# arkworks-rs/crypto-primitives

Measured on NVIDIA B200. Metric: poseidon_perms_per_sec, higher is better.
Workload: dtype u32x8 (256-bit Montgomery integer)

## Files before the change

### crypto_primitives_b200/csrc/cpb_poseidon.cu

```cuda
#include <cstdlib>
#include <vector>

#include "poseidon_kernels.cuh"

namespace cpb {

std::string& last_error_ref() {
    static thread_local std::string s;
    return s;
}
cpb_status fail(cpb_status st, const char* fmt, ...) {
    char buf[512];
    va_list ap;
    va_start(ap, fmt);
    vsnprintf(buf, sizeof buf, fmt, ap);
    va_end(ap);
    last_error_ref() = buf;
    return st;
}
void keep_pool_memory(int device) {
    cudaMemPool_t pool = nullptr;
    if (cudaDeviceGetDefaultMemPool(&pool, device) == cudaSuccess && pool) {
        unsigned long long keep = ~0ull;
        cudaMemPoolSetAttribute(pool, cudaMemPoolAttrReleaseThreshold, &keep);
    }
    cudaGetLastError();
}
int sm_count(int device) {
    static int cache[64];
    static std::mutex mu;
    std::lock_guard<std::mutex> g(mu);
    if (device < 0 || device >= 64) return 148;
    if (!cache[device]) {
        int v = 0;
        if (cudaDeviceGetAttribute(&v, cudaDevAttrMultiProcessorCount, device) != cudaSuccess || v <= 0) v = 148;
        cache[device] = v;
    }
    return cache[device];
}

template <class F>
__global__ void k_field_convert(const u32* __restrict__ in, u32* __restrict__ out, long n, int to_mont) {
    long i = (long)blockIdx.x * blockDim.x + threadIdx.x;
    if (i >= n) return;
    u32 a[8], k[8];
    ld_elem(a, in + 8 * i);
    if (to_mont) {
        for (int it = 0; it < 18; it++) {
            u32 t[8];
            t[0] = sub_cc(a[0], F::P(0));
#pragma unroll
            for (int j = 1; j < 8; j++) t[j] = subc_cc(a[j], F::P(j));
            u32 borrow = subc(0, 0);
            if (borrow) break;
            fp_copy(a, t);
        }
#pragma unroll
        for (int j = 0; j < 8; j++) k[j] = F::R2(j);
    } else {
        fp_zero(k);
        k[0] = 1;
    }
    u32 pm[8];
    fp_modulus<F>(pm);
    fp_mul<F>(a, a, k, pm);
    st_elem(out + 8 * i, a);
}

}

using namespace cpb;

using namespace cpb;

namespace cpb {
CPB_POS_WIDTHS(CPB_POS_EXTERN, Bls12_381_Fr)
CPB_POS_WIDTHS(CPB_POS_EXTERN, Bn254_Fr)
CPB_POS_WIDTHS(CPB_POS_EXTERN, Jubjub_Fr)
CPB_POS_WIDTHS(CPB_POS_EXTERN, Bls12_377_Fr)
CPB_POS_EXTERN_TEAM(Bls12_381_Fr)
CPB_POS_EXTERN_TEAM(Bn254_Fr)
CPB_POS_EXTERN_TEAM(Jubjub_Fr)
CPB_POS_EXTERN_TEAM(Bls12_377_Fr)
}

namespace {

PoseidonDev to_dev(const host::PoseidonSchedule& S) {
    PoseidonDev D;
    D.t = S.t; D.rate = S.rate; D.cap = S.capacity; D.rf = S.rf; D.rp = S.rp; D.sparse = S.sparse; D.alpha = S.alpha;
    D.off_c = S.off_c; D.off_m = S.off_m; D.off_mpre = S.off_mpre; D.off_cp0 = S.off_cp0; D.off_pc = S.off_pc;
    D.off_sp = S.off_sp; D.off_arkp = S.off_arkp; D.off_mod = S.off_mod; D.off_sc0 = S.off_sc0; D.n_elems = S.n_elems; D.zero = 0;
    return D;
}


#define CPB_CASE_T(F, T, M, ...) case T: return M<F, T>(__VA_ARGS__);
#define CPB_FOR_T(F, M, ...)                                                                                   \
    switch (c->dev.t) {                                                                                        \
        CPB_CASE_T(F, 2, M, __VA_ARGS__) CPB_CASE_T(F, 3, M, __VA_ARGS__) CPB_CASE_T(F, 4, M, __VA_ARGS__)     \
        CPB_CASE_T(F, 5, M, __VA_ARGS__) CPB_CASE_T(F, 6, M, __VA_ARGS__) CPB_CASE_T(F, 7, M, __VA_ARGS__)     \
        CPB_CASE_T(F, 8, M, __VA_ARGS__) CPB_CASE_T(F, 9, M, __VA_ARGS__)                                      \
    }                                                                                                          \
    break;
#define CPB_FOR_FIELD(M, ...)                                                        \
    switch (c->field_id) {                                                           \
        case CPB_BLS12_381_FR: CPB_FOR_T(Bls12_381_Fr, M, __VA_ARGS__)               \
        case CPB_BN254_FR: CPB_FOR_T(Bn254_Fr, M, __VA_ARGS__)                       \
        case CPB_JUBJUB_FR: CPB_FOR_T(Jubjub_Fr, M, __VA_ARGS__)                     \
        case CPB_BLS12_377_FR: CPB_FOR_T(Bls12_377_Fr, M, __VA_ARGS__)               \
    }

size_t team_max() {
    static long v = -1;
    if (v < 0) {
        const char* e = getenv("CPB_TEAM_MAX");
        v = e ? atol(e) : 4096;
        if (v > 4096) v = 4096;
        if (v < 0) v = 0;
    }
    return (size_t)v;
}
size_t team_max_for(size_t S) {
    if (getenv("CPB_TEAM_MAX")) return team_max();
    size_t v = 8192 / (S ? S : 1);
    return v < team_max() ? v : team_max();
}
bool team_capable(const cpb_poseidon_ctx* c) { return c->dev.t == 3 && c->dev.cap == 1 && c->dev.alpha >= 2; }

cpb_status launch_tree_top(cpb_poseidon_ctx* c, const TopJob& J, cudaStream_t st) {
    switch (c->field_id) {
        case CPB_BLS12_381_FR: return launch_tree_top_f<Bls12_381_Fr>(c, J, st);
        case CPB_BN254_FR: return launch_tree_top_f<Bn254_Fr>(c, J, st);
        case CPB_JUBJUB_FR: return launch_tree_top_f<Jubjub_Fr>(c, J, st);
        case CPB_BLS12_377_FR: return launch_tree_top_f<Bls12_377_Fr>(c, J, st);
    }
    return fail(CPB_BAD_PARAMS, "unknown field id %d", c->field_id);
}

}

namespace cpb {
cpb_status launch_crh(cpb_poseidon_ctx* c, const u32* in, size_t len, u32* out, size_t n, cudaStream_t st, size_t n_out) {
    if (n == 0 || n_out == 0) return CPB_OK;
    if (team_capable(c) && len == 2 && n_out == 1 && n <= team_max()) {
        TopJob J;
        J.flat_in = in; J.flat_out = out; J.n_flat = (long)n;
        return launch_tree_top(c, J, st);
    }
    CPB_FOR_FIELD(launch_crh_ft, c, in, len, out, n_out, n, st)
    return fail(CPB_UNSUPPORTED, "state width t=%d is not built (this library: t = 2..9)", c->dev.t);
}
}

namespace {
cpb_status launch_verify(cpb_poseidon_ctx* c, cpb_poseidon_ctx* node, const u32* root, const u32* leaves, size_t leaf_len,
                         const u32* siblings, const u32* paths, int plen, const unsigned long long* indexes, unsigned char* ok,
                         size_t n, cudaStream_t st) {
    if (n == 0) return CPB_OK;
    CPB_FOR_FIELD(launch_verify_ft, c, node, root, leaves, leaf_len, siblings, paths, plen, indexes, ok, n, st)
    return fail(CPB_UNSUPPORTED, "state width t=%d is not built (this library: t = 2..9)", c->dev.t);
}
cpb_status launch_permute(cpb_poseidon_ctx* c, const u32* in, u32* out, size_t n, cudaStream_t st) {
    if (n == 0) return CPB_OK;
    CPB_FOR_FIELD(launch_permute_ft, c, in, out, n, st)
    return fail(CPB_UNSUPPORTED, "state width t=%d is not built (this library: t = 2..9)", c->dev.t);
}

}

namespace cpb {

cpb_status check_ctx(const cpb_poseidon_ctx* c) {
    if (!c) return fail(CPB_NULL_POINTER, "null context");
    return CPB_OK;
}

cpb_status merkle_subtree_levels(cpb_poseidon_ctx* node, const u32* leaf_digests, size_t n, u32* nodes, size_t S, size_t k,
                                 cudaStream_t st, const MerkleHost* H, const ExchangeDev* X, int* small_from) {
    int h = 0;
    while (((size_t)1 << h) < n) h++;
    int lg = 0;
    while (((size_t)1 << lg) < S) lg++;
    const bool team = team_capable(node) && team_max() > 0;
    const size_t tmax = team_max_for(S);
    for (int l = h - 1; l >= lg; l--) {
        size_t cnt = ((size_t)1 << l) / S;
        if (team && cnt <= tmax) {
            TopJob J;
            J.leaf_digests = leaf_digests; J.nodes = nodes; J.h = h; J.lgS = lg; J.k = (long)k; J.l_start = l; J.l_end = lg;
            if (X && S == 1) J.x = *X;
            CPB_TRY(launch_tree_top(node, J, st));
            if (small_from) *small_from = l;
            else if (H)
                for (int q = l; q >= lg; q--) {
                    size_t c2 = ((size_t)1 << q) / S, off = (((size_t)1 << q) - 1) + k * c2;
                    CPB_CUDA(cudaMemcpyAsync(H->node_ptr(q, k * c2), nodes + 8 * off, c2 * 32, cudaMemcpyDeviceToHost, st));
                }
            return CPB_OK;
        }
        const u32* in = (l == h - 1) ? leaf_digests + 8 * (2 * k * cnt) : nodes + 8 * ((((size_t)1 << (l + 1)) - 1) + 2 * k * cnt);
        u32* out = nodes + 8 * ((((size_t)1 << l) - 1) + k * cnt);
        CPB_TRY(launch_crh(node, in, 2, out, cnt, st));
        if (H) CPB_CUDA(cudaMemcpyAsync(H->node_ptr(l, k * cnt), out, cnt * 32, cudaMemcpyDeviceToHost, st));
    }
    if (X && S == 1) return fail(CPB_UNSUPPORTED, "the fused root exchange needs a rate-2, capacity-1 Poseidon two-to-one hash with alpha >= 2");
    return CPB_OK;
}
cpb_status merkle_levels(cpb_poseidon_ctx* node, const u32* leaf_digests, size_t n, u32* nodes, cudaStream_t st) {
    return merkle_subtree_levels(node, leaf_digests, n, nodes, 1, 0, st);
}

size_t merkle_streams(size_t n) {
    static int forced = -1;
    if (forced < 0) {
        const char* e = getenv("CPB_MERKLE_STREAMS");
        forced = e ? atoi(e) : 0;
    }
    size_t S = forced > 0 ? (size_t)forced : 8;
    if (S > 8) S = 8;
    while (S & (S - 1)) S &= S - 1;
    while (S > 1 && n / S < ((size_t)1 << 14)) S >>= 1;
    return S;
}

cpb_status ensure_side_streams(cpb_poseidon_ctx* c, size_t S) {
    std::lock_guard<std::mutex> lk(c->side_mu);
    for (size_t i = 0; i < S; i++)
        if (!c->side[i]) CPB_CUDA(cudaStreamCreateWithFlags(&c->side[i], cudaStreamNonBlocking));
    return CPB_OK;
}

cpb_status merkle_build_streams(cpb_poseidon_ctx* leaf, cpb_poseidon_ctx* node, const u32* leaves, size_t leaf_len, size_t n,
                                u32* leaf_nodes, u32* nodes, cudaStream_t st, const MerkleHost* H, const ExchangeDev* X) {
    size_t S = merkle_streams(n);
    if (S <= 1) {
        if (H && H->leaves && n * leaf_len) CPB_CUDA(cudaMemcpyAsync((void*)leaves, H->leaves, n * leaf_len * 32, cudaMemcpyHostToDevice, st));
        if (leaves) CPB_TRY(launch_crh(leaf, leaves, leaf_len, leaf_nodes, n, st));
        CPB_TRY(merkle_subtree_levels(node, leaf_nodes, n, nodes, 1, 0, st, H, X));
        if (H) CPB_CUDA(cudaMemcpyAsync(H->leaf_nodes, leaf_nodes, n * 32, cudaMemcpyDeviceToHost, st));
        return CPB_OK;
    }
    CPB_TRY(ensure_side_streams(node, S));
    int small_from = -1;
    cudaEvent_t start = nullptr, done[8] = {};
    CPB_CUDA(cudaEventCreateWithFlags(&start, cudaEventDisableTiming));
    cudaError_t e = cudaEventRecord(start, st);
    cpb_status rc = CPB_OK;
// ... 103 lines not shown
    if (!ptr) return fail(CPB_NULL_POINTER, "null buffer");
    CPB_CUDA(cudaHostUnregister(ptr));
    return CPB_OK;
    });
}

cpb_status cpb_field_modulus(int field_id, uint64_t out[4]) {
    return cpb::guarded([&]() -> cpb_status {
    const uint64_t* m = host::field_modulus(field_id);
    if (!m) return fail(CPB_BAD_PARAMS, "unknown field id %d", field_id);
    if (!out) return fail(CPB_NULL_POINTER, "null out");
    memcpy(out, m, 32);
    return CPB_OK;
    });
}

static cpb_status field_convert(int field_id, int device, const uint64_t* in, uint64_t* out, size_t n, int to_mont) {
    if (!host::field_modulus(field_id)) return fail(CPB_BAD_PARAMS, "unknown field id %d", field_id);
    if (n == 0) return CPB_OK;
    if (!in || !out) return fail(CPB_NULL_POINTER, "null buffer");
    DeviceGuard g(device);
    if (!g.ok) return fail(CPB_NO_DEVICE, "cudaSetDevice(%d) failed", device);
    u32* d = nullptr;
    CPB_CUDA(cudaMalloc(&d, n * 32));
    cudaError_t e = cudaMemcpy(d, in, n * 32, cudaMemcpyHostToDevice);
    if (e == cudaSuccess) {
        int grid = (int)((n + 127) / 128);
        switch (field_id) {
            case 0: k_field_convert<Bls12_381_Fr><<<grid, 128>>>(d, d, (long)n, to_mont); break;
            case 1: k_field_convert<Bn254_Fr><<<grid, 128>>>(d, d, (long)n, to_mont); break;
            case 2: k_field_convert<Jubjub_Fr><<<grid, 128>>>(d, d, (long)n, to_mont); break;
            case 3: k_field_convert<Bls12_377_Fr><<<grid, 128>>>(d, d, (long)n, to_mont); break;
        }
        e = cudaGetLastError();
    }
    if (e == cudaSuccess) e = cudaMemcpy(out, d, n * 32, cudaMemcpyDeviceToHost);
    cudaFree(d);
    if (e != cudaSuccess) return fail(CPB_CUDA_ERROR, "field conversion failed: %s", cudaGetErrorString(e));
    return CPB_OK;
}
static cpb_status field_convert_dev(int field_id, int device, const uint64_t* in, uint64_t* out, size_t n, int to_mont, void* stream) {
    if (!host::field_modulus(field_id)) return fail(CPB_BAD_PARAMS, "unknown field id %d", field_id);
    if (n == 0) return CPB_OK;
    if (!in || !out) return fail(CPB_NULL_POINTER, "null buffer");
    DeviceGuard g(device);
    if (!g.ok) return fail(CPB_NO_DEVICE, "cudaSetDevice(%d) failed", device);
    cudaStream_t st = (cudaStream_t)stream;
    const u32* d_in = (const u32*)in;
    u32* d_out = (u32*)out;
    long left = (long)n, off = 0;
    while (left > 0) {
        long m = left < (1L << 28) ? left : (1L << 28);
        int grid = (int)((m + 127) / 128);
        switch (field_id) {
            case 0: k_field_convert<Bls12_381_Fr><<<grid, 128, 0, st>>>(d_in + 8 * off, d_out + 8 * off, m, to_mont); break;
            case 1: k_field_convert<Bn254_Fr><<<grid, 128, 0, st>>>(d_in + 8 * off, d_out + 8 * off, m, to_mont); break;
            case 2: k_field_convert<Jubjub_Fr><<<grid, 128, 0, st>>>(d_in + 8 * off, d_out + 8 * off, m, to_mont); break;
            case 3: k_field_convert<Bls12_377_Fr><<<grid, 128, 0, st>>>(d_in + 8 * off, d_out + 8 * off, m, to_mont); break;
        }
        CPB_CUDA(cudaGetLastError());
        left -= m; off += m;
    }
    return CPB_OK;
}
cpb_status cpb_field_to_montgomery_dev(int field_id, int device, const uint64_t* in, uint64_t* out, size_t n, void* stream) {
    return cpb::guarded([&]() -> cpb_status { return field_convert_dev(field_id, device, in, out, n, 1, stream); });
}
cpb_status cpb_field_from_montgomery_dev(int field_id, int device, const uint64_t* in, uint64_t* out, size_t n, void* stream) {
    return cpb::guarded([&]() -> cpb_status { return field_convert_dev(field_id, device, in, out, n, 0, stream); });
}
cpb_status cpb_field_to_montgomery(int field_id, int device, const uint64_t* in, uint64_t* out, size_t n) {
    return cpb::guarded([&]() -> cpb_status {
    return field_convert(field_id, device, in, out, n, 1);
    });
}
cpb_status cpb_field_from_montgomery(int field_id, int device, const uint64_t* in, uint64_t* out, size_t n) {
    return cpb::guarded([&]() -> cpb_status {
    return field_convert(field_id, device, in, out, n, 0);
    });
}

cpb_status cpb_poseidon_find_ark_and_mds(int field_id, uint64_t prime_bits, int rate, int full_rounds,
                                         int partial_rounds, int skip_matrices, uint64_t* ark_out, uint64_t* mds_out) {
    return cpb::guarded([&]() -> cpb_status {
    const uint64_t* mod = host::field_modulus(field_id);
    if (!mod) return fail(CPB_BAD_PARAMS, "unknown field id %d", field_id);
    if (!ark_out || !mds_out) return fail(CPB_NULL_POINTER, "null output");
    host::Field F(mod);
    if (prime_bits != (uint64_t)F.bits)
        return fail(CPB_BAD_PARAMS, "prime_bits %llu != MODULUS_BIT_SIZE %d", (unsigned long long)prime_bits, F.bits);
    if (rate < 1 || rate > 15 || full_rounds < 0 || partial_rounds < 0 || full_rounds > 1023 || partial_rounds > 1023 ||
        skip_matrices < 0)
        return fail(CPB_BAD_PARAMS, "bad shape");
    host::FeVec ark, mds;
    host::find_poseidon_ark_and_mds(F, prime_bits, rate, full_rounds, partial_rounds, skip_matrices, ark, mds);
    memcpy(ark_out, ark.data(), ark.size() * 32);
    memcpy(mds_out, mds.data(), mds.size() * 32);
    return CPB_OK;
    });
}

cpb_status cpb_poseidon_default_entry(int field_id, int rate, int optimized_for_weights, uint64_t* alpha, int* full_rounds,
                                      int* partial_rounds, int* skip_matrices) {
    return cpb::guarded([&]() -> cpb_status {
    host::DefaultEntry e;
    if (!host::default_entry(field_id, rate, optimized_for_weights != 0, e))
        return fail(CPB_BAD_PARAMS, "no default entry for field %d rate %d", field_id, rate);
    if (alpha) *alpha = e.alpha;
    if (full_rounds) *full_rounds = e.rf;
    if (partial_rounds) *partial_rounds = e.rp;
    if (skip_matrices) *skip_matrices = e.skip;
    return CPB_OK;
    });
}

cpb_status cpb_poseidon_ctx_create(int field_id, int rate, int capacity, int full_rounds, int partial_rounds,
                                   uint64_t alpha, const uint64_t* ark, const uint64_t* mds, int device,
                                   cpb_poseidon_ctx** out) {
    return cpb::guarded([&]() -> cpb_status {
    if (!out) return fail(CPB_NULL_POINTER, "null out");
    *out = nullptr;
    const uint64_t* mod = host::field_modulus(field_id);
    if (!mod) return fail(CPB_BAD_PARAMS, "unknown field id %d", field_id);
    if (!ark || !mds) return fail(CPB_NULL_POINTER, "null ark/mds");
    if (rate < 1 || capacity < 1 || rate + capacity > 16 || full_rounds < 0 || partial_rounds < 0 ||
        full_rounds + partial_rounds < 1)
        return fail(CPB_BAD_PARAMS, "bad Poseidon shape rate=%d capacity=%d RF=%d RP=%d", rate, capacity, full_rounds,
                    partial_rounds);
    host::Field F(mod);
    host::PoseidonParams P;
    P.rate = rate; P.capacity = capacity; P.full_rounds = full_rounds; P.partial_rounds = partial_rounds; P.alpha = alpha;
    int t = rate + capacity;
    P.ark.resize((size_t)(full_rounds + partial_rounds) * t);
    P.mds.resize((size_t)t * t);
    memcpy(P.ark.data(), ark, P.ark.size() * 32);
    memcpy(P.mds.data(), mds, P.mds.size() * 32);
    for (const auto& e : P.ark)
        if (!F.is_canonical(e)) return fail(CPB_BAD_PARAMS, "ark element not reduced");
    for (const auto& e : P.mds)
        if (!F.is_canonical(e)) return fail(CPB_BAD_PARAMS, "mds element not reduced");

    DeviceGuard g(device);
    if (!g.ok) { cudaGetLastError(); return fail(CPB_NO_DEVICE, "cudaSetDevice(%d) failed: no usable CUDA device", device); }
    int major = 0;
    CPB_CUDA(cudaDeviceGetAttribute(&major, cudaDevAttrComputeCapabilityMajor, device));
    if (major != 10) return fail(CPB_NO_DEVICE, "device %d is sm_%d0; this library is built for sm_100a only", device, major);

    keep_pool_memory(device);
    cpb_poseidon_ctx* c = new cpb_poseidon_ctx();
    c->field_id = field_id;
    c->device = device;
    c->sms = sm_count(device);
    c->sched = host::derive_schedule(F, P, true);
    c->dev = to_dev(c->sched);
    size_t bytes = c->sched.consts.size() * 8;
    if (bytes > 200 * 1024) { delete c; return fail(CPB_UNSUPPORTED, "round schedule (%zu B) exceeds shared memory", bytes); }
    cudaError_t e = cudaMalloc(&c->d_consts, bytes);
    if (e == cudaSuccess) e = cudaMemcpy(c->d_consts, c->sched.consts.data(), bytes, cudaMemcpyHostToDevice);
    if (e == cudaSuccess) e = cudaStreamCreateWithFlags(&c->stream, cudaStreamNonBlocking);
    if (e != cudaSuccess) {
        if (c->d_consts) cudaFree(c->d_consts);
        delete c;
        return fail(CPB_CUDA_ERROR, "context upload failed: %s", cudaGetErrorString(e));
    }
    *out = c;
    return CPB_OK;
    });
}

void cpb_poseidon_ctx_destroy(cpb_poseidon_ctx* c) {
    if (!c) return;
    DeviceGuard g(c->device);
    if (c->stream) { cudaStreamSynchronize(c->stream); cudaStreamDestroy(c->stream); }
    if (c->d_consts) cudaFree(c->d_consts);
    for (auto& s : c->side)
        if (s) { cudaStreamSynchronize(s); cudaStreamDestroy(s); }
    c->s_in.release(); c->s_out.release(); c->s_aux.release();
    delete c;
}

int cpb_poseidon_ctx_is_sparse(const cpb_poseidon_ctx* c) { return c ? c->sched.sparse : 0; }
int cpb_poseidon_ctx_field(const cpb_poseidon_ctx* c) { return c ? c->field_id : -1; }
int cpb_poseidon_ctx_device(const cpb_poseidon_ctx* c) { return c ? c->device : -1; }

cpb_status cpb_poseidon_permute_batch_dev(cpb_poseidon_ctx* c, const uint64_t* in, uint64_t* out, size_t n, void* stream) {
    return cpb::guarded([&]() -> cpb_status {
    CPB_TRY(check_ctx(c));
    DeviceGuard g(c->device);
    return launch_permute(c, (const u32*)in, (u32*)out, n, (cudaStream_t)stream);
    });
}
cpb_status cpb_poseidon_crh_batch_dev(cpb_poseidon_ctx* c, const uint64_t* in, size_t len, uint64_t* out, size_t n, void* stream) {
    return cpb::guarded([&]() -> cpb_status {
    CPB_TRY(check_ctx(c));
    DeviceGuard g(c->device);
    return launch_crh(c, (const u32*)in, len, (u32*)out, n, (cudaStream_t)stream);
    });
}
cpb_status cpb_poseidon_sponge_batch_dev(cpb_poseidon_ctx* c, const uint64_t* in, size_t len, uint64_t* out, size_t n_squeeze,
                                         size_t n, void* stream) {
    return cpb::guarded([&]() -> cpb_status {
    CPB_TRY(check_ctx(c));
    DeviceGuard g(c->device);
    return launch_crh(c, (const u32*)in, len, (u32*)out, n, (cudaStream_t)stream, n_squeeze);
    });
}
cpb_status cpb_merkle_poseidon_verify_batch_dev(cpb_poseidon_ctx* leaf, cpb_poseidon_ctx* node, const uint64_t* root,
                                                const uint64_t* leaves, size_t leaf_len, const uint64_t* leaf_sibling_hashes,
                                                const uint64_t* auth_paths, size_t path_len, const uint64_t* leaf_indexes,
                                                uint8_t* ok, size_t n, void* stream) {
    return cpb::guarded([&]() -> cpb_status {
    CPB_TRY(check_ctx(leaf));
    CPB_TRY(check_ctx(node));
    if (leaf->device != node->device || leaf->field_id != node->field_id || leaf->dev.t != node->dev.t)
        return fail(CPB_UNSUPPORTED, "leaf and node contexts must share device, field and state width");
    if (node->dev.rate < 2) return fail(CPB_UNSUPPORTED, "two-to-one with rate < 2 not supported");
    if (path_len > 62) return fail(CPB_BAD_PARAMS, "path too long");
    DeviceGuard g(leaf->device);
    return launch_verify(leaf, node, (const u32*)root, (const u32*)leaves, leaf_len, (const u32*)leaf_sibling_hashes,
                         (const u32*)auth_paths, (int)path_len, (const unsigned long long*)leaf_indexes, ok, n, (cudaStream_t)stream);
    });
}
cpb_status cpb_poseidon_compress_batch_dev(cpb_poseidon_ctx* c, const uint64_t* pairs, uint64_t* out, size_t n, void* stream) {
    return cpb::guarded([&]() -> cpb_status {
    CPB_TRY(check_ctx(c));
    if (c->dev.rate < 2)
        return fail(CPB_UNSUPPORTED, "two-to-one with rate < 2 not supported");
    DeviceGuard g(c->device);
    return launch_crh(c, (const u32*)pairs, 2, (u32*)out, n, (cudaStream_t)stream);
    });
}
cpb_status cpb_merkle_poseidon_from_digests_dev(cpb_poseidon_ctx* node, const uint64_t* leaf_digests, size_t n,
                                                uint64_t* non_leaf_nodes, void* stream) {
    return cpb::guarded([&]() -> cpb_status {
    CPB_TRY(check_ctx(node));
    if (!pow2_gt1(n)) return fail(CPB_NOT_POW2, "leaves.len() should be power of two and greater than one (got %zu)", n);
    if (node->dev.rate < 2) return fail(CPB_UNSUPPORTED, "two-to-one with rate < 2 not supported");
    DeviceGuard g(node->device);
    return merkle_build_streams(node, node, nullptr, 0, n, (u32*)leaf_digests, (u32*)non_leaf_nodes, (cudaStream_t)stream);
    });
}
cpb_status cpb_merkle_poseidon_build_dev(cpb_poseidon_ctx* leaf, cpb_poseidon_ctx* node, const uint64_t* leaves,
                                         size_t leaf_len, size_t n, uint64_t* leaf_nodes, uint64_t* non_leaf_nodes,
                                         void* stream) {
    return cpb::guarded([&]() -> cpb_status {
    CPB_TRY(check_ctx(leaf));
    CPB_TRY(check_ctx(node));
    if (leaf->device != node->device || leaf->field_id != node->field_id)
        return fail(CPB_BAD_PARAMS, "leaf and node contexts must share device and field");
    if (!pow2_gt1(n)) return fail(CPB_NOT_POW2, "leaves.len() should be power of two and greater than one (got %zu)", n);
    if (node->dev.rate < 2) return fail(CPB_UNSUPPORTED, "two-to-one with rate < 2 not supported");
    DeviceGuard g(leaf->device);
    return merkle_build_streams(leaf, node, (const u32*)leaves, leaf_len, n, (u32*)leaf_nodes, (u32*)non_leaf_nodes,
                                (cudaStream_t)stream);
    });
}

static cpb_status host_roundtrip_crh(cpb_poseidon_ctx* c, const uint64_t* in, size_t in_elems_per, size_t len,
                                     uint64_t* out, size_t out_elems_per, size_t n, int mode) {
    CPB_TRY(check_ctx(c));
    if (n == 0) return CPB_OK;
    if ((!in && in_elems_per) || !out) return fail(CPB_NULL_POINTER, "null buffer");
    std::lock_guard<std::mutex> lk(c->mu);
    DeviceGuard g(c->device);
    size_t in_b = n * in_elems_per * 32, out_b = n * out_elems_per * 32;
    CPB_TRY(c->s_in.reserve(in_b ? in_b : 32));
    CPB_TRY(c->s_out.reserve(out_b));
    if (in_b) CPB_CUDA(cudaMemcpyAsync(c->s_in.ptr, in, in_b, cudaMemcpyHostToDevice, c->stream));
    if (mode == 0) CPB_TRY(launch_crh(c, (const u32*)c->s_in.ptr, len, (u32*)c->s_out.ptr, n, c->stream));
    else CPB_TRY(launch_permute(c, (const u32*)c->s_in.ptr, (u32*)c->s_out.ptr, n, c->stream));
    CPB_CUDA(cudaMemcpyAsync(out, c->s_out.ptr, out_b, cudaMemcpyDeviceToHost, c->stream));
    CPB_CUDA(cudaStreamSynchronize(c->stream));
    return CPB_OK;
}
cpb_status cpb_poseidon_permute_batch(cpb_poseidon_ctx* c, const uint64_t* in, uint64_t* out, size_t n) {
    return cpb::guarded([&]() -> cpb_status {
    CPB_TRY(check_ctx(c));
    return host_roundtrip_crh(c, in, (size_t)c->dev.t, 0, out, (size_t)c->dev.t, n, 1);
    });
}
cpb_status cpb_poseidon_crh_batch(cpb_poseidon_ctx* c, const uint64_t* in, size_t len, uint64_t* out, size_t n) {
    return cpb::guarded([&]() -> cpb_status {
    return host_roundtrip_crh(c, in, len, len, out, 1, n, 0);
    });
}
cpb_status cpb_poseidon_sponge_batch(cpb_poseidon_ctx* c, const uint64_t* in, size_t len, uint64_t* out, size_t n_squeeze, size_t n) {
    return cpb::guarded([&]() -> cpb_status {
    CPB_TRY(check_ctx(c));
    if (n == 0 || n_squeeze == 0) return CPB_OK;
    if ((!in && len) || !out) return fail(CPB_NULL_POINTER, "null buffer");
    std::lock_guard<std::mutex> lk(c->mu);
    DeviceGuard g(c->device);
    size_t in_b = n * len * 32, out_b = n * n_squeeze * 32;
    CPB_TRY(c->s_in.reserve(in_b ? in_b : 32));
    CPB_TRY(c->s_out.reserve(out_b));
    if (in_b) CPB_CUDA(cudaMemcpyAsync(c->s_in.ptr, in, in_b, cudaMemcpyHostToDevice, c->stream));
    CPB_TRY(launch_crh(c, (const u32*)c->s_in.ptr, len, (u32*)c->s_out.ptr, n, c->stream, n_squeeze));
    CPB_CUDA(cudaMemcpyAsync(out, c->s_out.ptr, out_b, cudaMemcpyDeviceToHost, c->stream));
    CPB_CUDA(cudaStreamSynchronize(c->stream));
    return CPB_OK;
    });
}
cpb_status cpb_merkle_poseidon_verify_batch(cpb_poseidon_ctx* leaf, cpb_poseidon_ctx* node, const uint64_t* root,
                                            const uint64_t* leaves, size_t leaf_len, const uint64_t* leaf_sibling_hashes,
                                            const uint64_t* auth_paths, size_t path_len, const uint64_t* leaf_indexes, uint8_t* ok,
                                            size_t n) {
    return cpb::guarded([&]() -> cpb_status {
// ... 81 lines not shown
```

### crypto_primitives_b200/csrc/poseidon.cuh

```cuda
#pragma once
#include "fp.cuh"

namespace cpb {

struct PoseidonDev {
    int t, rate, cap, rf, rp, sparse;
    u64 alpha;
    int off_c, off_m, off_mpre, off_cp0, off_pc, off_sp, off_arkp, off_mod, off_sc0, n_elems;
    int zero;
};

template <class F, int T> CPB_HD void pos_add_vec(u32 (&s)[T][8], const u32* c) {
#pragma unroll
    for (int i = 0; i < T; i++) {
        u32 k[8];
        ld_elem(k, c + 8 * i);
        fp_add<F>(s[i], s[i], k);
    }
}

template <int T> CPB_HD void pos_rotl(u32 (&s)[T][8]) {
    u32 tmp[8];
    fp_copy(tmp, s[0]);
#pragma unroll
    for (int i = 0; i + 1 < T; i++) fp_copy(s[i], s[i + 1]);
    fp_copy(s[T - 1], tmp);
}

template <class F> CPB_HD void pos_sbox(u32* x, u64 alpha, int top_bit, const u32* pm, bool lazy = false) {
    u32 x0[8];
    fp_copy(x0, x);
#pragma unroll 1
    for (int i = top_bit - 1; i >= 0; i--) {
        if constexpr (F::LAZY5) {
            fp_sqr_rt<F>(x, x, pm, lazy);
            if ((alpha >> i) & 1) fp_mul_rt<F>(x, x, x0, pm, lazy);
        } else {
            fp_sqr<F>(x, x, pm);
            if ((alpha >> i) & 1) fp_mul<F>(x, x, x0, pm);
        }
    }
}

#ifdef CPB_POS_SPLIT
#define CPB_POS_SPLIT_FOR(F) (CPB_POS_SPLIT != 0)
#else
#define CPB_POS_SPLIT_FOR(F) (F::SPLIT_ROUNDS)
#endif
#ifndef CPB_SBOX5
#define CPB_SBOX5 1
#endif
#ifndef CPB_COL_UNROLL_MAX
#define CPB_COL_UNROLL_MAX 4
#endif

struct PermuteHint {
    int lane0_zero;
    unsigned need;
};

template <class F, int T> CPB_HD void pos_permute_split(u32 (&s)[T][8], const PoseidonDev& P, const u32* cs, const u32* pm, const PermuteHint& H) {
    const int half = P.rf / 2;
    int top_bit = 0;
    for (int i = 63; i > 0; i--)
        if ((P.alpha >> i) & 1) { top_bit = i; break; }
    const bool alpha_zero = P.alpha == 0;
    constexpr bool LZ = F::LAZY5 && !detail::dot_needs_x<F, T + 1>() && T <= 4;
    static_assert(!F::LAZY5 || 100 * ((u64)F::P(7) + 1) <= 19 * ((u64)1 << LIMB_BITS), "LAZY5 needs p/2^256 <= 0.19");
    const bool lazy = LZ && CPB_SBOX5 && P.alpha == 5;
    u32 n[T][8];
#pragma unroll
    for (int i = 0; i < T; i++) fp_zero(n[i]);
#pragma unroll 1
    for (int phase = 0; phase < 2; phase++) {
        const int cnt = phase == 0 ? half : P.rf - half;
#pragma unroll 1
        for (int q = 0; q < cnt; q++) {
            pos_add_vec<F, T>(s, cs + 8 * (P.off_c + (phase * half + q) * T));
            const int first_j = (H.lane0_zero != 0 && phase == 0 && q == 0) ? 0 : -1;
            const unsigned need = (phase == 1 && q == cnt - 1) ? H.need : ~0u;
#pragma unroll 1
            for (int j = 0; j < T; j++) {
                if (j == first_j) ld_elem(s[0], cs + 8 * P.off_sc0);
                else if (alpha_zero) fp_one<F>(s[0]);
                else pos_sbox<F>(s[0], P.alpha, top_bit, pm, lazy);
                pos_rotl<T>(s);
            }
            const u32* rows = cs + 8 * ((phase == 0 && q == half - 1) ? P.off_mpre : P.off_m);
#pragma unroll 1
            for (int i = 0; i < T; i++) {
                u32 d[8];
                fp_zero(d);
                if ((need >> i) & 1u) fp_dot<F, T, LZ ? 1 : 0>(d, s, rows + 8 * T * i, pm);
#pragma unroll
                for (int k = 0; k + 1 < T; k++) fp_copy(n[k], n[k + 1]);
                fp_copy(n[T - 1], d);
            }
#pragma unroll
            for (int i = 0; i < T; i++) fp_copy(s[i], n[i]);
        }
        if (phase == 0 && P.rp > 0) {
            pos_add_vec<F, T>(s, cs + 8 * P.off_cp0);
            const u32* row = cs + 8 * P.off_sp;
            const u32* pc = cs + 8 * (P.off_pc + 1);
#pragma unroll 1
            for (int k = 0; k < P.rp; k++, row += 8 * (2 * T - 1), pc += 8) {
#if CPB_SBOX5
                if (P.alpha == 5) {
                    u32 x2[8];
                    fp_sqr<F, LZ>(x2, s[0], pm);
                    fp_sqr<F, LZ>(x2, x2, pm);
                    fp_mul<F, LZ>(s[0], x2, s[0], pm);
                } else
#endif
                if (alpha_zero) fp_one<F>(s[0]);
                else pos_sbox<F>(s[0], P.alpha, top_bit, pm);
                u32 d[8];
                fp_dot<F, T, LZ ? 1 : 0>(d, s, row, pm);
                const u32* v = row + 8 * T;
                if (T <= CPB_COL_UNROLL_MAX) {
#pragma unroll
                    for (int j = 1; j < T; j++) {
                        u32 c[8], tmp[8];
                        ld_elem(c, v + 8 * (j - 1));
                        fp_mul<F>(tmp, s[0], c, pm);
                        fp_add<F>(s[j], s[j], tmp);
                    }
                } else {
#pragma unroll 1
                    for (int j = 1; j < T; j++) {
                        u32 c[8], tmp[8];
                        ld_elem(c, v + 8 * (j - 1));
                        fp_mul<F>(tmp, s[0], c, pm);
                        fp_add<F>(s[1], s[1], tmp);
                        fp_copy(tmp, s[1]);
#pragma unroll
                        for (int q = 1; q + 1 < T; q++) fp_copy(s[q], s[q + 1]);
                        fp_copy(s[T - 1], tmp);
                    }
                }
                if (k + 1 < P.rp) {
                    u32 c[8];
                    ld_elem(c, pc);
                    if (lazy) fp_add_noreduce(s[0], d, c);
                    else fp_add<F>(s[0], d, c);
                } else {
                    fp_copy(s[0], d);
                }
            }
        }
    }
}

template <class F, int T> CPB_HD void pos_permute(u32 (&s)[T][8], const PoseidonDev& P, const u32* cs, const u32* pm,
                                                  const PermuteHint& H = PermuteHint{0, ~0u}) {
    if constexpr (CPB_POS_SPLIT_FOR(F)) {
        if (P.sparse) {
            pos_permute_split<F, T>(s, P, cs, pm, H);
            return;
        }
    }
    const int half = P.rf / 2, total = P.rf + P.rp;
    int top_bit = 0;
    for (int i = 63; i > 0; i--)
        if ((P.alpha >> i) & 1) { top_bit = i; break; }
    const bool alpha_zero = P.alpha == 0;
    u32 n[T][8];
#pragma unroll
    for (int i = 0; i < T; i++) fp_zero(n[i]);
#pragma unroll 1
    for (int r = 0; r < total; r++) {
        const bool full = r < half || r >= half + P.rp;
        const int k = r - half;
        if (full) {
            const int fr = r < half ? r : r - P.rp;
            pos_add_vec<F, T>(s, cs + 8 * (P.off_c + fr * T));
        } else if (!P.sparse) {
            pos_add_vec<F, T>(s, cs + 8 * (P.off_arkp + k * T));
        } else if (k == 0) {
            pos_add_vec<F, T>(s, cs + 8 * P.off_cp0);
        }
        const int lanes = full ? T : 1;
#pragma unroll 1
        for (int j = 0; j < lanes; j++) {
            if (alpha_zero) fp_one<F>(s[0]);
            else pos_sbox<F>(s[0], P.alpha, top_bit, pm);
            if (full) pos_rotl<T>(s);
        }
        const bool dense = full || !P.sparse;
        const u32* rows = dense ? cs + 8 * ((full && r == half - 1) ? P.off_mpre : P.off_m)
                                : cs + 8 * (P.off_sp + k * (2 * T - 1));
        const int nrows = dense ? T : 1;
        u32 d[8];
#pragma unroll 1
        for (int i = 0; i < nrows; i++) {
            fp_dot<F, T>(d, s, rows + 8 * T * i, pm);
            if (dense) {
#pragma unroll
                for (int q = 0; q + 1 < T; q++) fp_copy(n[q], n[q + 1]);
                fp_copy(n[T - 1], d);
            }
        }
        if (dense) {
#pragma unroll
            for (int i = 0; i < T; i++) fp_copy(s[i], n[i]);
        } else {
            const u32* v = rows + 8 * T;
            if (T <= CPB_COL_UNROLL_MAX) {
#pragma unroll
                for (int j = 1; j < T; j++) {
                    u32 c[8], tmp[8];
                    ld_elem(c, v + 8 * (j - 1));
                    fp_mul<F>(tmp, s[0], c, pm);
                    fp_add<F>(s[j], s[j], tmp);
                }
            } else {
#pragma unroll 1
                for (int j = 1; j < T; j++) {
                    u32 c[8], tmp[8];
                    ld_elem(c, v + 8 * (j - 1));
                    fp_mul<F>(tmp, s[0], c, pm);
                    fp_add<F>(s[1], s[1], tmp);
                    fp_copy(tmp, s[1]);
#pragma unroll
                    for (int q = 1; q + 1 < T; q++) fp_copy(s[q], s[q + 1]);
                    fp_copy(s[T - 1], tmp);
                }
            }
            if (k + 1 < P.rp) {
                u32 c[8];
                ld_elem(c, cs + 8 * (P.off_pc + k + 1));
                fp_add<F>(s[0], d, c);
            } else {
                fp_copy(s[0], d);
            }
        }
    }
}

template <class F, int T>
CPB_HD void pos_sponge(u32* out, long n_out, const u32* in, long len, const PoseidonDev& P, const u32* cs, const u32* pm) {
    u32 s[T][8];
#pragma unroll
    for (int i = 0; i < T; i++) fp_zero(s[i]);
    const int rate = P.rate, cap = P.cap;
    const long nblocks = len <= rate ? 1 : (len + rate - 1) / rate;
    const long nsq = n_out <= rate ? 1 : (n_out + rate - 1) / rate;
#pragma unroll 1
    for (long b = 0; b < nblocks + nsq - 1; b++) {
        if (b < nblocks) {
            const long pos = b * rate;
            const long rem = len - pos;
            const int cnt = rem > rate ? rate : (int)rem;
#pragma unroll
            for (int i = 0; i < T; i++) {
// ... 71 lines not shown
```

### crypto_primitives_b200/csrc/poseidon_host.hpp

```cpp
#pragma once
#include "hostfp.hpp"

namespace cpb {
namespace host {

class GrainLFSR {
public:
    GrainLFSR(bool sbox_inverse, u64 prime_bits, u64 state_len, u64 rf, u64 rp) : prime_bits_(prime_bits) {
        for (int i = 0; i < 80; i++) st_[i] = 0;
        st_[1] = 1;
        st_[5] = sbox_inverse ? 1 : 0;
        put(6, 17, prime_bits);
        put(18, 29, state_len);
        put(30, 39, rf);
        put(40, 49, rp);
        for (int i = 50; i < 80; i++) st_[i] = 1;
        head_ = 0;
        for (int i = 0; i < 160; i++) update();
    }

    void draw(u64 out[4]) {
        out[0] = out[1] = out[2] = out[3] = 0;
        for (u64 i = 0; i < prime_bits_; i++) {
            u64 bitpos = prime_bits_ - 1 - i;
            if (next_filtered_bit()) out[bitpos / 64] |= 1ull << (bitpos % 64);
        }
    }

    FeVec rejection_sampling(const Field& F, size_t n) {
        FeVec r;
        while (r.size() < n) {
            u64 v[4];
            draw(v);
            if (!Field::geq(v, F.p)) r.push_back(F.from_canonical(v));
        }
        return r;
    }
    FeVec mod_p(const Field& F, size_t n) {
        FeVec r;
        for (size_t i = 0; i < n; i++) {
            u64 v[4];
            draw(v);
            r.push_back(F.from_canonical(v));
        }
        return r;
    }

private:
    void put(int lo, int hi, u64 v) {
        for (int i = hi; i >= lo; i--) { st_[i] = v & 1; v >>= 1; }
    }
    int update() {
        int nb = st_[(head_ + 62) % 80] ^ st_[(head_ + 51) % 80] ^ st_[(head_ + 38) % 80] ^
                 st_[(head_ + 23) % 80] ^ st_[(head_ + 13) % 80] ^ st_[head_];
        st_[head_] = (unsigned char)nb;
        head_ = (head_ + 1) % 80;
        return nb;
    }
    int next_filtered_bit() {
        int b = update();
        while (!b) { update(); b = update(); }
        return update();
    }
    unsigned char st_[80];
    int head_;
    u64 prime_bits_;
};

struct PoseidonParams {
    int rate = 0, capacity = 0, full_rounds = 0, partial_rounds = 0;
    u64 alpha = 0;
    FeVec ark;
    FeVec mds;
    int t() const { return rate + capacity; }
};

inline void find_poseidon_ark_and_mds(const Field& F, u64 prime_bits, int rate, int rf, int rp, int skip,
                                      FeVec& ark, FeVec& mds) {
    int t = rate + 1;
    GrainLFSR lfsr(false, prime_bits, (u64)t, (u64)rf, (u64)rp);
    ark.clear();
    for (int r = 0; r < rf + rp; r++) {
        FeVec row = lfsr.rejection_sampling(F, (size_t)t);
        ark.insert(ark.end(), row.begin(), row.end());
    }
    for (int s = 0; s < skip; s++) (void)lfsr.mod_p(F, (size_t)(2 * t));
    FeVec xs = lfsr.mod_p(F, (size_t)t), ys = lfsr.mod_p(F, (size_t)t);
    mds.assign((size_t)t * t, F.zero());
    for (int i = 0; i < t; i++)
        for (int j = 0; j < t; j++) mds[(size_t)i * t + j] = F.inv(F.add(xs[i], ys[j]));
}

struct DefaultEntry { int rate; u64 alpha; int rf, rp, skip; };
inline bool default_entry(int field_id, int rate, bool optimized_for_weights, DefaultEntry& e) {
    if (field_id != 0) return false;
    static const DefaultEntry C[7] = {{2, 17, 8, 31, 0}, {3, 5, 8, 56, 0}, {4, 5, 8, 56, 0}, {5, 5, 8, 57, 0},
                                      {6, 5, 8, 57, 0},  {7, 5, 8, 57, 0}, {8, 5, 8, 57, 0}};
    if (rate < 2 || rate > 8) return false;
    if (optimized_for_weights) e = DefaultEntry{rate, 257, 8, 13, 0};
    else e = C[rate - 2];
    return true;
}

struct PoseidonSchedule {
    int t = 0, rate = 0, capacity = 0, rf = 0, rp = 0, sparse = 0;
    u64 alpha = 0;
    int off_c = 0;
    int off_m = 0;
    int off_mpre = 0;
    int off_cp0 = 0;
    int off_pc = 0;
    int off_sp = 0;
    int off_arkp = 0;
    int off_mod = 0;
    int off_sc0 = 0;
    int n_elems = 0;
    std::vector<u64> consts;
};

namespace detail {
inline FeVec matmul(const Field& F, const FeVec& A, const FeVec& B, int n) {
    FeVec C((size_t)n * n, F.zero());
    for (int i = 0; i < n; i++)
        for (int j = 0; j < n; j++) {
            Fe acc = F.zero();
            for (int k = 0; k < n; k++) acc = F.add(acc, F.mul(A[(size_t)i * n + k], B[(size_t)k * n + j]));
            C[(size_t)i * n + j] = acc;
        }
    return C;
}
inline FeVec matvec(const Field& F, const FeVec& A, const FeVec& x, int n) {
    FeVec y((size_t)n, F.zero());
    for (int i = 0; i < n; i++) {
        Fe acc = F.zero();
        for (int k = 0; k < n; k++) acc = F.add(acc, F.mul(A[(size_t)i * n + k], x[k]));
        y[i] = acc;
    }
    return y;
}
inline bool invert(const Field& F, FeVec A, int m, FeVec& out) {
    FeVec I((size_t)m * m, F.zero());
    for (int i = 0; i < m; i++) I[(size_t)i * m + i] = F.one();
    for (int c = 0; c < m; c++) {
        int piv = -1;
        for (int r = c; r < m; r++)
            if (!A[(size_t)r * m + c].is_zero()) { piv = r; break; }
        if (piv < 0) return false;
        if (piv != c)
            for (int k = 0; k < m; k++) {
                std::swap(A[(size_t)piv * m + k], A[(size_t)c * m + k]);
                std::swap(I[(size_t)piv * m + k], I[(size_t)c * m + k]);
            }
        Fe inv = F.inv(A[(size_t)c * m + c]);
        for (int k = 0; k < m; k++) {
            A[(size_t)c * m + k] = F.mul(A[(size_t)c * m + k], inv);
            I[(size_t)c * m + k] = F.mul(I[(size_t)c * m + k], inv);
        }
        for (int r = 0; r < m; r++) {
            if (r == c) continue;
            Fe f = A[(size_t)r * m + c];
            if (f.is_zero()) continue;
            for (int k = 0; k < m; k++) {
                A[(size_t)r * m + k] = F.sub(A[(size_t)r * m + k], F.mul(f, A[(size_t)c * m + k]));
                I[(size_t)r * m + k] = F.sub(I[(size_t)r * m + k], F.mul(f, I[(size_t)c * m + k]));
            }
        }
    }
    out = I;
    return true;
}
}

inline PoseidonSchedule derive_schedule(const Field& F, const PoseidonParams& P, bool allow_sparse = true) {
    const int t = P.t(), rf = P.full_rounds, rp = P.partial_rounds, half = rf / 2;
    PoseidonSchedule S;
    S.t = t; S.rate = P.rate; S.capacity = P.capacity; S.rf = rf; S.rp = rp; S.alpha = P.alpha;

    const FeVec& M = P.mds;
    FeVec C((size_t)rf * t), Mpre = M, Cp0((size_t)t, F.zero()), pc((size_t)(rp > 0 ? rp : 1), F.zero());
    FeVec sp((size_t)(rp > 0 ? rp : 1) * (2 * t - 1), F.zero()), arkp;
    auto ark = [&](int r, int i) -> const Fe& { return P.ark[(size_t)r * t + i]; };
    for (int fr = 0; fr < rf; fr++) {
        int r = fr < half ? fr : half + rp + (fr - half);
        for (int i = 0; i < t; i++) C[(size_t)fr * t + i] = ark(r, i);
    }
    for (int k = 0; k < rp; k++)
        for (int i = 0; i < t; i++) arkp.push_back(ark(half + k, i));

    bool sparse = allow_sparse && rp > 0 && t >= 2 && half >= 1 && rf > half;
    if (sparse) {
        FeVec D((size_t)t * t, F.zero());
        for (int i = 0; i < t; i++) D[(size_t)i * t + i] = F.one();
        const int m = t - 1;
        for (int k = rp - 1; k >= 0 && sparse; k--) {
            FeVec N = detail::matmul(F, D, M, t);
            FeVec Mhat((size_t)m * m), Minv;
            for (int i = 0; i < m; i++)
                for (int j = 0; j < m; j++) Mhat[(size_t)i * m + j] = N[(size_t)(i + 1) * t + (j + 1)];
            if (!detail::invert(F, Mhat, m, Minv)) { sparse = false; break; }
            for (int j = 0; j < m; j++) {
                Fe acc = F.zero();
                for (int i = 0; i < m; i++) acc = F.add(acc, F.mul(N[(size_t)0 * t + (i + 1)], Minv[(size_t)i * m + j]));
                sp[(size_t)k * (2 * t - 1) + 1 + j] = acc;
            }
            sp[(size_t)k * (2 * t - 1)] = N[0];
            for (int i = 0; i < m; i++) sp[(size_t)k * (2 * t - 1) + t + i] = N[(size_t)(i + 1) * t + 0];
            for (auto& e : D) e = F.zero();
            D[0] = F.one();
            for (int i = 0; i < m; i++)
                for (int j = 0; j < m; j++) D[(size_t)(i + 1) * t + (j + 1)] = Mhat[(size_t)i * m + j];
        }
        if (sparse) {
            Mpre = detail::matmul(F, D, M, t);
            FeVec c0((size_t)t);
            for (int i = 0; i < t; i++) c0[i] = ark(half, i);
            Cp0 = detail::matvec(F, D, c0, t);
            FeVec d((size_t)t, F.zero());
            for (int k = 1; k < rp; k++) {
                FeVec md = detail::matvec(F, M, d, t);
                FeVec cp((size_t)t);
                for (int i = 0; i < t; i++) cp[i] = F.add(ark(half + k, i), md[i]);
                pc[k] = cp[0];
                d = cp;
                d[0] = F.zero();
            }
            FeVec post = detail::matvec(F, M, d, t);
            if (rf > half)
                for (int i = 0; i < t; i++) C[(size_t)half * t + i] = F.add(C[(size_t)half * t + i], post[i]);
            else sparse = false;
        }
    }
    if (!sparse) {
        for (int fr = 0; fr < rf; fr++) {
            int r = fr < half ? fr : half + rp + (fr - half);
            for (int i = 0; i < t; i++) C[(size_t)fr * t + i] = ark(r, i);
        }
        Mpre = M;
    }
    S.sparse = sparse ? 1 : 0;

    auto push = [&](const FeVec& v) {
        int off = (int)(S.consts.size() / 4);
        for (const Fe& e : v) S.consts.insert(S.consts.end(), e.l, e.l + 4);
        return off;
    };
    S.off_c = push(C);
    S.off_m = push(M);
    S.off_mpre = push(Mpre);
    S.off_cp0 = push(Cp0);
    S.off_pc = push(pc);
    S.off_sp = push(sp);
    if (sparse) arkp.clear();
    S.off_arkp = push(arkp);
    {
        Fe pm;
        memcpy(pm.l, F.p, 32);
        S.off_mod = push(FeVec(1, pm));
    }
    {
        Fe y = F.one(), b = C.empty() ? F.zero() : C[0];
        for (u64 e = P.alpha; e; e >>= 1) {
            if (e & 1) y = F.mul(y, b);
            b = F.mul(b, b);
        }
        S.off_sc0 = push(FeVec(1, y));
    }
    S.n_elems = (int)(S.consts.size() / 4);
    return S;
}

}
}
```

Baseline: 130.1 million.

## Add width-3 partial-round recurrence to replace sparse matrix partial rounds

For t=3 sparse schedules, the host derives a linear recurrence expressing each partial round's new lane-0 value as a 5-term dot product over the last few S-box outputs and previous values. It also derives a final reconstruction of lanes 1 and 2 from that history. The device runs this recurrence in place of the sparse-matrix partial rounds, so each round needs one 5-term dot instead of updating every lane. The change adds host-side Gaussian elimination, keeps more state in registers, and also zeroes the accumulator before each full-round MDS.

```diff
diff --git a/crypto_primitives_b200/csrc/cpb_poseidon.cu b/crypto_primitives_b200/csrc/cpb_poseidon.cu
--- a/crypto_primitives_b200/csrc/cpb_poseidon.cu
+++ b/crypto_primitives_b200/csrc/cpb_poseidon.cu
@@ -85,15 +85,6 @@
 }
 
 namespace {
-
-PoseidonDev to_dev(const host::PoseidonSchedule& S) {
-    PoseidonDev D;
-    D.t = S.t; D.rate = S.rate; D.cap = S.capacity; D.rf = S.rf; D.rp = S.rp; D.sparse = S.sparse; D.alpha = S.alpha;
-    D.off_c = S.off_c; D.off_m = S.off_m; D.off_mpre = S.off_mpre; D.off_cp0 = S.off_cp0; D.off_pc = S.off_pc;
-    D.off_sp = S.off_sp; D.off_arkp = S.off_arkp; D.off_mod = S.off_mod; D.off_sc0 = S.off_sc0; D.n_elems = S.n_elems; D.zero = 0;
-    return D;
-}
-
 
 #define CPB_CASE_T(F, T, M, ...) case T: return M<F, T>(__VA_ARGS__);
 #define CPB_FOR_T(F, M, ...)                                                                                   \
@@ -503,7 +494,7 @@
     c->device = device;
     c->sms = sm_count(device);
     c->sched = host::derive_schedule(F, P, true);
-    c->dev = to_dev(c->sched);
+    c->dev = host::make_dev(c->sched);
     size_t bytes = c->sched.consts.size() * 8;
     if (bytes > 200 * 1024) { delete c; return fail(CPB_UNSUPPORTED, "round schedule (%zu B) exceeds shared memory", bytes); }
     cudaError_t e = cudaMalloc(&c->d_consts, bytes);
diff --git a/crypto_primitives_b200/csrc/poseidon.cuh b/crypto_primitives_b200/csrc/poseidon.cuh
--- a/crypto_primitives_b200/csrc/poseidon.cuh
+++ b/crypto_primitives_b200/csrc/poseidon.cuh
@@ -8,6 +8,7 @@
     u64 alpha;
     int off_c, off_m, off_mpre, off_cp0, off_pc, off_sp, off_arkp, off_mod, off_sc0, n_elems;
     int zero;
+    int recur = 0, off_rc = 0, off_rk = 0, off_rr = 0;
 };
 
 template <class F, int T> CPB_HD void pos_add_vec(u32 (&s)[T][8], const u32* c) {
@@ -53,11 +54,61 @@
 #ifndef CPB_COL_UNROLL_MAX
 #define CPB_COL_UNROLL_MAX 4
 #endif
+#ifndef CPB_POS_RECUR
+#define CPB_POS_RECUR 1
+#endif
 
 struct PermuteHint {
     int lane0_zero;
     unsigned need;
 };
+
+template <class F, bool LZ> CPB_HD void pos_partial_recur(u32 (&s)[3][8], const PoseidonDev& P, const u32* cs, const u32* pm, bool lazy,
+                                                          int top_bit) {
+    constexpr int EXH = LZ ? 4 : 0, EXR = LZ ? 3 : 0;
+    const bool alpha_zero = P.alpha == 0;
+    u32 h[5][8];
+    fp_copy(h[1], s[1]);
+    fp_copy(h[2], s[2]);
+    fp_copy(h[3], s[0]);
+    fp_zero(h[4]);
+    const u32* row = cs + 8 * P.off_rc;
+    const u32* ck = cs + 8 * P.off_rk;
+#pragma unroll 1
+    for (int k = 0; k < P.rp; k++, ck += 8) {
+        fp_copy(h[0], h[3]);
+#if CPB_SBOX5
+        if (P.alpha == 5) {
+            u32 x2[8];
+            fp_sqr<F, LZ>(x2, h[0], pm);
+            fp_sqr<F, LZ>(x2, x2, pm);
+            fp_mul<F, LZ>(h[0], x2, h[0], pm);
+        } else
+#endif
+        if (alpha_zero) fp_one<F>(h[0]);
+        else pos_sbox<F>(h[0], P.alpha, top_bit, pm);
+        u32 d[8], c[8];
+        fp_dot<F, 5, EXH>(d, h, row, pm);
+        if (k < 2) row += 8 * 5;
+        ld_elem(c, ck);
+        fp_copy(h[2], h[1]);
+        fp_copy(h[1], h[0]);
+        fp_copy(h[4], h[3]);
+        if (lazy && k + 1 < P.rp) fp_add_noreduce(h[3], d, c);
+        else fp_add<F>(h[3], d, c);
+    }
+    u32 g[4][8], c[8];
+#pragma unroll
+    for (int i = 0; i < 4; i++) fp_copy(g[i], h[i + 1]);
+    const u32* rr = cs + 8 * P.off_rr;
+    fp_copy(s[0], h[3]);
+    fp_dot<F, 4, EXR>(s[1], g, rr, pm);
+    ld_elem(c, rr + 8 * 8);
+    fp_add<F>(s[1], s[1], c);
+    fp_dot<F, 4, EXR>(s[2], g, rr + 8 * 4, pm);
+    ld_elem(c, rr + 8 * 9);
+    fp_add<F>(s[2], s[2], c);
+}
 
 template <class F, int T> CPB_HD void pos_permute_split(u32 (&s)[T][8], const PoseidonDev& P, const u32* cs, const u32* pm, const PermuteHint& H) {
     const int half = P.rf / 2;
@@ -87,6 +138,8 @@
                 pos_rotl<T>(s);
             }
             const u32* rows = cs + 8 * ((phase == 0 && q == half - 1) ? P.off_mpre : P.off_m);
+#pragma unroll
+            for (int i = 0; i < T; i++) fp_zero(n[i]);
 #pragma unroll 1
             for (int i = 0; i < T; i++) {
                 u32 d[8];
@@ -101,6 +154,12 @@
         }
         if (phase == 0 && P.rp > 0) {
             pos_add_vec<F, T>(s, cs + 8 * P.off_cp0);
+            if constexpr (T == 3 && CPB_POS_RECUR != 0) {
+                if (P.recur) {
+                    pos_partial_recur<F, LZ>(s, P, cs, pm, lazy, top_bit);
+                    continue;
+                }
+            }
             const u32* row = cs + 8 * P.off_sp;
             const u32* pc = cs + 8 * (P.off_pc + 1);
 #pragma unroll 1
diff --git a/crypto_primitives_b200/csrc/poseidon_host.hpp b/crypto_primitives_b200/csrc/poseidon_host.hpp
--- a/crypto_primitives_b200/csrc/poseidon_host.hpp
+++ b/crypto_primitives_b200/csrc/poseidon_host.hpp
@@ -1,5 +1,8 @@
 #pragma once
+#include <algorithm>
+
 #include "hostfp.hpp"
+#include "poseidon.cuh"
 
 namespace cpb {
 namespace host {
@@ -114,6 +117,10 @@
     int off_arkp = 0;
     int off_mod = 0;
     int off_sc0 = 0;
+    int recur = 0;
+    int off_rc = 0;
+    int off_rk = 0;
+    int off_rr = 0;
     int n_elems = 0;
     std::vector<u64> consts;
 };
@@ -167,6 +174,88 @@
         }
     }
     out = I;
+    return true;
+}
+
+inline FeVec form_var(const Field& F, int nv, int v) {
+    FeVec f((size_t)nv, F.zero());
+    if (v >= 0) f[(size_t)v] = F.one();
+    return f;
+}
+inline void form_axpy(const Field& F, FeVec& r, const Fe& c, const FeVec& a) {
+    for (size_t i = 0; i < r.size(); i++) r[i] = F.add(r[i], F.mul(c, a[i]));
+}
+inline bool solve_affine(const Field& F, const FeVec& f, const std::vector<FeVec>& g, FeVec& c, Fe& k) {
+    const int n = (int)g.size(), rows = (int)f.size() - 1;
+    std::vector<FeVec> A((size_t)rows, FeVec((size_t)n + 1));
+    for (int v = 0; v < rows; v++) {
+        for (int i = 0; i < n; i++) A[v][i] = g[i][(size_t)v + 1];
+        A[v][n] = f[(size_t)v + 1];
+    }
+    std::vector<int> pivcol;
+    int r = 0;
+    for (int col = 0; col < n && r < rows; col++) {
+        int piv = -1;
+        for (int q = r; q < rows; q++)
+            if (!A[q][col].is_zero()) { piv = q; break; }
+        if (piv < 0) continue;
+        std::swap(A[piv], A[r]);
+        const Fe inv = F.inv(A[r][col]);
+        for (auto& e : A[r]) e = F.mul(e, inv);
+        for (int q = 0; q < rows; q++) {
+            if (q == r || A[q][col].is_zero()) continue;
+            const Fe m = A[q][col];
+            for (int i = 0; i <= n; i++) A[q][i] = F.sub(A[q][i], F.mul(m, A[r][i]));
+        }
+        pivcol.push_back(col);
+        r++;
+    }
+    for (int q = r; q < rows; q++)
+        if (!A[q][n].is_zero()) return false;
+    c.assign((size_t)n, F.zero());
+    for (int j = 0; j < r; j++) c[(size_t)pivcol[j]] = A[j][n];
+    k = f[0];
+    for (int i = 0; i < n; i++) k = F.sub(k, F.mul(c[i], g[i][0]));
+    return true;
+}
+
+inline bool derive_recurrence(const Field& F, int rp, const FeVec& sp, const FeVec& pc, FeVec& rows, FeVec& ck, FeVec& rr) {
+    const int w = 5, nv = 4 + rp;
+    if (rp < 3) return false;
+    auto var = [&](int v) { return form_var(F, nv, v); };
+    FeVec l1 = var(1), l2 = var(2);
+    std::vector<FeVec> x{var(3)};
+    for (int k = 0; k < rp; k++) {
+        const Fe* row = &sp[(size_t)k * w];
+        const FeVec y = var(4 + k);
+        FeVec d((size_t)nv, F.zero());
+        form_axpy(F, d, row[0], y);
+        form_axpy(F, d, row[1], l1);
+        form_axpy(F, d, row[2], l2);
+        form_axpy(F, l1, row[3], y);
+        form_axpy(F, l2, row[4], y);
+        if (k + 1 < rp) d[0] = F.add(d[0], pc[(size_t)k + 1]);
+        x.push_back(d);
+    }
+    rows.clear(); ck.clear(); rr.clear();
+    for (int k = 0; k < rp; k++) {
+        const std::vector<FeVec> h{var(4 + k), var(k >= 1 ? 3 + k : 1), var(k >= 2 ? 2 + k : k == 1 ? 1 : 2), x[(size_t)k],
+                                   k >= 1 ? x[(size_t)k - 1] : var(-1)};
+        FeVec c;
+        Fe c0;
+        if (!solve_affine(F, x[(size_t)k + 1], h, c, c0)) return false;
+        if (k <= 2) rows.insert(rows.end(), c.begin(), c.end());
+        else if (!std::equal(c.begin(), c.end(), rows.begin() + 2 * w)) return false;
+        ck.push_back(c0);
+    }
+    const std::vector<FeVec> h{var(3 + rp), var(2 + rp), x[(size_t)rp], x[(size_t)rp - 1]};
+    FeVec c1, c2;
+    Fe k1, k2;
+    if (!solve_affine(F, l1, h, c1, k1) || !solve_affine(F, l2, h, c2, k2)) return false;
+    rr = c1;
+    rr.insert(rr.end(), c2.begin(), c2.end());
+    rr.push_back(k1);
+    rr.push_back(k2);
     return true;
 }
 }
@@ -265,9 +354,25 @@
         }
         S.off_sc0 = push(FeVec(1, y));
     }
+    FeVec rrows, rk, rr;
+    if (sparse && t == 3 && detail::derive_recurrence(F, rp, sp, pc, rrows, rk, rr)) {
+        S.recur = 1;
+        S.off_rc = push(rrows);
+        S.off_rk = push(rk);
+        S.off_rr = push(rr);
+    }
     S.n_elems = (int)(S.consts.size() / 4);
     return S;
 }
 
-}
-}
+inline PoseidonDev make_dev(const PoseidonSchedule& S) {
+    PoseidonDev D;
+    D.t = S.t; D.rate = S.rate; D.cap = S.capacity; D.rf = S.rf; D.rp = S.rp; D.sparse = S.sparse; D.alpha = S.alpha;
+    D.off_c = S.off_c; D.off_m = S.off_m; D.off_mpre = S.off_mpre; D.off_cp0 = S.off_cp0; D.off_pc = S.off_pc;
+    D.off_sp = S.off_sp; D.off_arkp = S.off_arkp; D.off_mod = S.off_mod; D.off_sc0 = S.off_sc0; D.n_elems = S.n_elems; D.zero = 0;
+    D.recur = S.recur; D.off_rc = S.off_rc; D.off_rk = S.off_rk; D.off_rr = S.off_rr;
+    return D;
+}
+
+}
+}
```

Measured after the change: 144.8 million, median of 6. 11.3% higher.
